# nucypher/TFHE.jl

Hardware: AMD Instinct MI355X
Metric: bootstrapped gates/sec (whole node), N=1024 (higher is better)
Workload: dtype int32 torus / f64 transform; 1 GPU; batch of 4096 independent gate_nand() bootstraps per GPU, tfhe_parameters_80 (n=500, N=1024, k=1, l=2, Bg=2^10, ks t=8, base 2^2); inputs=resident in HBM, launch=one process

## Files before the change

### tfhe.jl_amd/csrc/engine.hpp

```cpp
#pragma once
#include <hip/hip_runtime.h>

#include <algorithm>
#include <atomic>
#include <cstdarg>
#include <cstdio>
#include <cstring>
#include <new>
#include <string>
#include <thread>
#include <vector>

#include "../../include/tfhe_mi355x.h"
#include "experiment.hpp"
#include "br_core.hpp"

using namespace tfhe;

#include "kernels_blind_rotate.hpp"
#include "kernels_anyn.hpp"
#include "kernels_n512.hpp"
#include "kernels_keyswitch.hpp"

struct ErrBuf {
    char s[512] = {0};
    const char *c_str() const { return s; }
    void set(const char *msg) { snprintf(s, sizeof s, "%s", msg ? msg : ""); }
    ErrBuf &operator=(const char *msg) { set(msg); return *this; }
    void format(const char *fmt, ...) __attribute__((format(printf, 2, 3)))
    {
        va_list ap;
        va_start(ap, fmt);
        vsnprintf(s, sizeof s, fmt, ap);
        va_end(ap);
    }
};
extern thread_local ErrBuf g_create_error;

struct DevBuf {
    void *p = nullptr;
    size_t cap = 0;
    hipError_t reserve(size_t bytes)
    {
        if (bytes <= cap) return hipSuccess;
        if (p) (void)hipFree(p);
        p = nullptr; cap = 0;
        size_t want = bytes + bytes / 4 + 256;
        hipError_t e = hipMalloc(&p, want);
        if (e == hipSuccess) cap = want;
        return e;
    }
    void release() { if (p) (void)hipFree(p); p = nullptr; cap = 0; }
};

struct PairXfer {
    static constexpr int kSlots = 4;
    struct Slot {
        DevBuf out, idx_src;
        DevBuf in, idx_dst;
        int32_t *h_idx = nullptr; size_t h_idx_cap = 0;
        void *h_rows = nullptr; size_t h_rows_cap = 0;
        hipEvent_t ready = nullptr;
        hipEvent_t taken = nullptr;
        bool pending = false;
    } slot[kSlots];
    unsigned next = 0;
};

struct KsKey {
    int mode = 0;
    int parties = 1;
    int kN = 0;
    void *p = nullptr;
    size_t per_party = 0;
    int stride = 0;
    int wtiles = 0;
};
inline void release(KsKey &k)
{
    if (k.p) (void)hipFree(k.p);
    k = KsKey{};
}

struct tfhe_ctx {
    tfhe_params P{};
    int device = 0;
    ErrBuf err;
    std::vector<tfhe_ctx *> kids;
    std::vector<uint8_t> kid_ran;

    hipStream_t stream = nullptr;
    static constexpr int kTimingSlots = 33;
    hipEvent_t evring[kTimingSlots][4] = {};
    hipEvent_t *ev = evring[0];
    int64_t timed_calls = 0;
    hipEvent_t done_ev = nullptr;
    bool done_pending = false;
    bool timing_valid = false;
    bool own_pending = false;
    int64_t last_rotations = 0;
    std::string last_kernel;
    int ks_slices_large = 2;
    int ks_variant = 4;
    int64_t br_small = 1024;
    int br_prio_pct = 90;
    int br_general = 0;
    int br_split = 1;
    int timing_events = 1;
    int br_rt_l = 0;
    int64_t br_tiny = -2;

    cplx *d_tables = nullptr;
    Tables T{};
    Gadget g{};
    cplx *d_anyn_tab = nullptr;
    int br_anyn = 0;
    int anyn_spec = -1;
    bool anyn() const
    {
        if (br_anyn) return true;
        if (P.parties > 1) return P.N != kN || P.parties > 8 || P.bs_l > 8;
        if (n512()) return false;
        return (P.N != kN && P.N != 2048) || P.k > 4;
    }
    bool n512() const { return !br_anyn && P.parties == 1 && P.N == 512 && P.k == 1; }

    cplx *d_bk = nullptr;       size_t bk_polys = 0;
    KsKey ks;
    bool have_bk = false;
    bool have_ks() const { return ks.mode != 0 && ks.parties == 1; }
    cplx *d_mk_bk = nullptr;
    int mk_parties = 0;
    bool have_mk_bk = false;
    bool have_mk_ks() const { return ks.mode != 0 && ks.parties > 1; }

    int32_t *d_wires = nullptr; int64_t num_wires = 0;
    int wires_parties = 0;
    size_t wire_words() const { return wires_parties ? (size_t)wires_parties * P.n + 1 : (size_t)P.n + 1; }

    DevBuf bara, ext, map, io[4], diag, abar, mk_acc, spec;
    DevBuf tv, tv_index;
    DevBuf tv_bodies, tv_ext;
    cplx *d_tgsw = nullptr;        int64_t tgsw_count = 0;
    DevBuf lvl_ws[2], lvl_data, lvl_spec;
    cplx *d_mk_tgsw = nullptr;     int64_t mk_tgsw_count = 0;
    int32_t *d_mk_tgsw_party = nullptr;
    size_t diag_rows = 0;
    bool mk_force_general = false;
    int n2048_rw = 0;
    int mkg_rw = 0;
    int mkg_variant = 0;
    int mkg_acc = -1;
    int mk_rw = 0;
    bool measure_margin = false;
    int exact_domain = 2;
    double exact_bound_log2 = 0;
    double exact_margin = 0;
    tfhe_ctx *twin = nullptr;
    std::atomic<hipStream_t> twin_stream{nullptr};
    bool borrows_keys = false;
    bool slot_busy[2] = {false, false};
    std::atomic<std::thread::id> submit_thread{};
    uint32_t submits = 0;
    std::vector<std::vector<uint8_t>> wire_valid;
    std::vector<int32_t> wire_owner;
    std::vector<uint8_t> peer_ok;
    std::vector<struct PairXfer *> xfer;
    int level_exchange = 0;
    int64_t level_split_min = 4096;
    std::vector<int32_t> kid_tickets[2];
    int cu_count = 256;
    int w2_rw = 0;
    int n512_w2 = -1;
    int n512_rw = 0;
    int k2_w3 = -1;
    int k2_rw = 0;
    int v3_rw = 0;
    int64_t pipeline_min = 4096;
    bool last_call_two_streams = false;
    struct MapStage { void *h = nullptr; size_t cap = 0; hipEvent_t ev = nullptr; bool pending = false; };
    static constexpr int kMapStages = 4;
    MapStage map_stage[kMapStages];
    unsigned map_next = 0;
    MapStage *map_cur = &map_stage[0];
    void *h_map = nullptr;
// ... 71 lines not shown
constexpr size_t kTan2TableOffset = kN512TableOffset + kN512TableElems;

inline int ilog2i(int x) { int r = 0; while ((1 << r) < x) r++; return r; }
inline bool op_has_a(int op) { return !(op == TFHE_GATE_CONST0 || op == TFHE_GATE_CONST1); }
inline bool op_has_b(int op) { return op_has_a(op) && !(op == TFHE_GATE_NOT || op == TFHE_GATE_COPY); }
inline size_t bk_poly_count(const tfhe_params &p) { return (size_t)p.n * p.bs_l * (p.k + 1) * (p.k + 1); }

template <typename F>
struct ScopeExit {
    F f;
    ~ScopeExit() { f(); }
};
template <typename F>
ScopeExit<F> on_exit(F f) { return ScopeExit<F>{f}; }

template <typename F>
static int32_t fan_out(tfhe_ctx *c, const std::vector<int> &which, F &&fn)
{
    std::vector<int32_t> rcs(which.size(), TFHE_OK);
    std::vector<std::thread> th;
    std::vector<size_t> inline_ones;
    th.reserve(which.size());
    inline_ones.reserve(which.size());
    auto shard = [&](size_t i) noexcept {
        try { rcs[i] = fn(which[i]); } catch (...) { rcs[i] = abi_caught(c->kids[(size_t)which[i]], "fan-out shard"); }
    };
    for (size_t i = 1; i < which.size(); i++) {
        try {
            th.emplace_back([&shard, i] { shard(i); });
        } catch (...) {
            inline_ones.push_back(i);
        }
    }
    if (!which.empty()) shard(0);
    for (size_t i : inline_ones) shard(i);
    for (auto &t : th) t.join();
    std::fill(c->kid_ran.begin(), c->kid_ran.end(), 0);
    for (int k : which) c->kid_ran[(size_t)k] = 1;
    for (size_t i = 0; i < which.size(); i++)
        if (rcs[i]) return c->set_err(rcs[i], "device %d (kid %d): %s", c->kids[(size_t)which[i]]->device, which[i], c->kids[(size_t)which[i]]->err.c_str());
    return TFHE_OK;
}
inline std::vector<int> all_kids(const tfhe_ctx *c)
{
    std::vector<int> v(c->kids.size());
    for (size_t i = 0; i < v.size(); i++) v[i] = (int)i;
    return v;
}

template <typename F>
static int32_t multi_rows(tfhe_ctx *c, int64_t B, F &&call)
{
    const int nk = (int)c->kids.size();
    std::vector<int> which;
    std::vector<int64_t> lo((size_t)nk), hi((size_t)nk);
    for (int r = 0; r < nk; r++) {
        lo[(size_t)r] = B * r / nk; hi[(size_t)r] = B * (r + 1) / nk;
        if (hi[(size_t)r] > lo[(size_t)r]) which.push_back(r);
    }
    return fan_out(c, which, [&](int r) { return call(c->kids[(size_t)r], lo[(size_t)r], hi[(size_t)r] - lo[(size_t)r]); });
}

void shard_bounds_by_rotations(const uint8_t *opcodes, int64_t B, int shards, int64_t *bounds);
void quiesce(tfhe_ctx *c);
int32_t tgsw_prepare(tfhe_ctx *c, const int32_t *d_polys, cplx *d_out, size_t npolys, hipStream_t s);
void mk_tgsw_drop(tfhe_ctx *c);
struct DiagArgs;
int32_t prepare_diag(tfhe_ctx *c, size_t R, hipStream_t s, DiagArgs &d);
void name_kernel(tfhe_ctx *c, const char *fmt, ...) __attribute__((format(printf, 2, 3)));
struct TvPtrs { const int32_t *tv; const int32_t *index; int32_t *bodies = nullptr; int32_t n_out = 1; };
template <class A>
static WithTv<A> with_tv(const A &a, const TvPtrs &tv)
{
    WithTv<A> t;
    static_cast<A &>(t) = a;
    t.tv = tv.tv;
    t.tv_index = tv.index;
    t.bodies = tv.bodies;
    t.n_out = tv.n_out;
    return t;
}
int32_t launch_blind_rotate(tfhe_ctx *c, size_t R, int32_t mu, hipStream_t s, const TvPtrs *tv = nullptr);
int32_t launch_keyswitch(tfhe_ctx *c, size_t G, const int32_t *e0, const int32_t *e1, const int32_t *dst, const int32_t *ext, int32_t *out, hipStream_t s);
int32_t enter_stream(tfhe_ctx *c, hipStream_t s);
int32_t leave_stream(tfhe_ctx *c, hipStream_t s);
void next_timing_slot(tfhe_ctx *c);
void commit_timing_slot(tfhe_ctx *c);
int32_t ensure_host_map(tfhe_ctx *c, size_t bytes);
int32_t launch_prologue(tfhe_ctx *c, size_t R, const int32_t *d_in0, const int32_t *d_in1, const int32_t *d_in2, const int32_t *d_ra, const int32_t *d_rb,
                        const uint8_t *d_kind, int words, hipStream_t s);
int32_t run_gates(tfhe_ctx *c, const char *who, const uint8_t *opcodes, int64_t B, const int32_t *d_in0, const int32_t *d_in1, const int32_t *d_in2,
                  int32_t *d_out, const int32_t *ia, const int32_t *ib, const int32_t *ic, const int32_t *io, hipStream_t s);
int32_t launch_linear_prologue(tfhe_ctx *c, bool lut, size_t B, const int32_t *d_start, const int32_t *d_wire, const int32_t *d_coef,
                               const int32_t *d_cst, const int32_t *d_out, hipStream_t s);
struct IntLevel {
    const int32_t *tv; int32_t n_tv; const int32_t *tv_index; int32_t n_out;
    const int32_t *term_start, *term_wire, *term_coef, *cst, *out;
    int64_t B;
};
int32_t run_int_level(tfhe_ctx *c, const IntLevel &L);
int32_t launch_trivial(tfhe_ctx *c, size_t T, const int32_t *d_in0, const int32_t *d_ts, const int32_t *d_td, const uint8_t *d_top, int32_t *d_out,
                       int words, hipStream_t s);
int32_t launch_mk_blind_rotate(tfhe_ctx *c, size_t R, hipStream_t s, const TvPtrs *tv = nullptr);
int32_t mk_tv_launch_anyn(tfhe_ctx *c, const WithTv<anyn::Args> &a, unsigned nblk, unsigned nt, size_t lds, hipStream_t s);
int32_t mk_tv_launch_w2(tfhe_ctx *c, const WithTv<MkBrArgs> &a, int rw, unsigned nblk, size_t lds, hipStream_t s);
int32_t mk_tv_launch_general(tfhe_ctx *c, const WithTv<MkGenArgs> &a, int rw, bool accg, unsigned nblk, size_t lds, hipStream_t s);
int32_t run_mk_gates(tfhe_ctx *c, const char *who, const uint8_t *opcodes, int64_t B, const int32_t *d_in0, const int32_t *d_in1, const int32_t *d_in2,
                     int32_t *d_out, const int32_t *ia, const int32_t *ib, const int32_t *ic, const int32_t *io, hipStream_t s);
struct BrLaunch {
    int L;
    int rw;
    bool dg;
    dim3 grid, block;
    size_t lds;
};
int32_t br_launch_anyn(tfhe_ctx *c, const WithTv<anyn::Args> &a, const BrLaunch &g, hipStream_t s);
int32_t br_launch_n512w2(tfhe_ctx *c, const WithTv<N512Args> &a, const BrLaunch &g, hipStream_t s);
int32_t br_launch_n512(tfhe_ctx *c, const WithTv<N512Args> &a, const BrLaunch &g, hipStream_t s);
int32_t br_launch_general(tfhe_ctx *c, const WithTv<BrGenArgs> &a, bool n2048, const BrLaunch &g, hipStream_t s);
int32_t br_launch_n2048x(tfhe_ctx *c, const WithTv<Br2048Args> &a, const BrLaunch &g, hipStream_t s);
int32_t br_launch_k2w3(tfhe_ctx *c, const WithTv<BrArgs> &a, const BrLaunch &g, hipStream_t s);
int32_t br_launch_k2(tfhe_ctx *c, const WithTv<BrArgs> &a, const BrLaunch &g, hipStream_t s);
int32_t br_launch_h2(tfhe_ctx *c, const WithTv<BrArgs> &a, const H2Tables &ht, const BrLaunch &g, hipStream_t s);
int32_t br_launch_w2(tfhe_ctx *c, const WithTv<BrArgs> &a, const BrLaunch &g, hipStream_t s);
int32_t br_launch_v3(tfhe_ctx *c, const WithTv<BrArgs> &a, const BrLaunch &g, hipStream_t s);
struct LvlWant { DevBuf *buf; size_t bytes; };
int32_t leveled_reserve(tfhe_ctx *c, const char *who, const LvlWant *want, int count);
int32_t pull_wires(tfhe_ctx *c, int dst, const int32_t *wires, int64_t count);
```

### tfhe.jl_amd/csrc/engine_diag.hip

```cpp
#include "engine.hpp"

int32_t tfhe_last_timing_ms(tfhe_ctx *c, int32_t which, float *ms) try
{
    ENTER_CTX(c);
    if (!c || !ms) return TFHE_ERR_INVALID_ARG;
    if (c->multi()) {
        float worst = -1.f;
        for (size_t k = 0; k < c->kids.size(); k++) {
            if (!c->kid_ran[k]) continue;
            float v = 0.f;
            const int32_t rc = tfhe_last_timing_ms(c->kids[k], which, &v);
            if (rc) { c->err = c->kids[k]->err; return rc; }
            worst = v > worst ? v : worst;
        }
        if (worst < 0.f) return c->set_err(TFHE_ERR_STATE, "last_timing: no batch call recorded");
        *ms = worst;
        return TFHE_OK;
    }
    if (!c->timing_valid) return c->set_err(TFHE_ERR_STATE, "last_timing: no batch call recorded");
    HIP_TRY(c, hipSetDevice(c->device));
    HIP_TRY(c, hipEventSynchronize(c->ev[3]));
    int a, b;
    switch (which) {
    case 0: a = 1; b = 2; break;
// ... 121 lines not shown
    }
    return TFHE_OK;
}

int32_t tfhe_last_rounding_margin(tfhe_ctx *c, double *worst) try
{
    ENTER_CTX(c);
    if (!c || !worst) return TFHE_ERR_INVALID_ARG;
    if (c->multi()) {
        double m = -1;
        for (size_t k = 0; k < c->kids.size(); k++) {
            if (!c->kid_ran[k]) continue;
            double v = 0;
            const int32_t rc = read_diag(c->kids[k], &v, nullptr);
            if (rc) { c->err = c->kids[k]->err; return rc; }
            m = v > m ? v : m;
        }
        if (m < 0) return c->set_err(TFHE_ERR_STATE, "last_rounding_margin: no batch call recorded");
        *worst = m;
        return TFHE_OK;
    }
    return read_diag(c, worst, nullptr);
}
ABI_CATCH(c, "tfhe_last_rounding_margin")

int32_t tfhe_last_kernel_clock_mhz(tfhe_ctx *c, double *mhz) try
{
    ENTER_CTX(c);
    if (!c || !mhz) return TFHE_ERR_INVALID_ARG;
    if (c->multi()) {
        for (size_t k = 0; k < c->kids.size(); k++) {
            if (!c->kid_ran[k]) continue;
            const int32_t rc = read_diag(c->kids[k], nullptr, mhz);
            if (rc) c->err = c->kids[k]->err;
            return rc;
        }
        return c->set_err(TFHE_ERR_STATE, "last_kernel_clock: no batch call recorded");
    }
    return read_diag(c, nullptr, mhz);
}
ABI_CATCH(c, "tfhe_last_kernel_clock_mhz")

#ifdef TFHE_STAMP
extern "C" int32_t tfhe_debug_phases(tfhe_ctx *c, unsigned long long *out64)
{
    if (!c || !out64 || c->multi() || !c->diag_rows) return TFHE_ERR_STATE;
    HIP_TRY(c, hipSetDevice(c->device));
    HIP_TRY(c, hipDeviceSynchronize());
    HIP_TRY(c, hipMemcpyAsync(out64, (const char *)c->diag.p + c->diag_rows * 24, 64 * 8, hipMemcpyDeviceToHost, c->stream));
    HIP_TRY(c, hipStreamSynchronize(c->stream));
    return TFHE_OK;
}
#endif

int32_t tfhe_get_option(tfhe_ctx *c, const char *name, int64_t *value) try
{
    if (!c && name && value && !strcmp(name, "debug_fail_alloc_after")) { *value = g_fail_alloc_countdown.load(); return TFHE_OK; }
    ENTER_CTX(c);
    if (!name || !value) return c->set_err(TFHE_ERR_INVALID_ARG, "get_option: NULL argument");
    if (!strcmp(name, "exact_domain")) { *value = c->exact_domain; return TFHE_OK; }
    if (!strcmp(name, "exact_bound_log2_x1000")) { *value = (int64_t)std::llround(c->exact_bound_log2 * 1000.0); return TFHE_OK; }
    if (!strcmp(name, "exact_margin_x1e6")) { *value = (int64_t)std::llround(c->exact_margin * 1e6); return TFHE_OK; }
    if (!strcmp(name, "debug_fail_alloc_after")) { *value = g_fail_alloc_countdown.load(); return TFHE_OK; }
    if (c->multi() && !strcmp(name, "peer_pairs")) {
        int64_t n = 0;
        const size_t nk = c->kids.size();
        for (size_t a = 0; a < nk; a++)
            for (size_t b = 0; b < nk; b++) n += (a != b && c->peer_ok[a * nk + b]) ? 1 : 0;
        *value = n;
        return TFHE_OK;
    }
    if (c->multi() && strcmp(name, "level_split_min") && strcmp(name, "level_exchange")) {
        const int32_t rc = tfhe_get_option(c->kids[0], name, value);
        if (rc) c->err = c->kids[0]->err;
        return rc;
    }
    const struct { const char *n; int64_t v; } table[] = {
        {"br_small", c->br_small}, {"br_tiny", c->br_tiny}, {"br_rt_l", c->br_rt_l}, {"timing_events", c->timing_events},
        {"br_split", c->br_split}, {"br_general", c->br_general}, {"br_anyn", c->br_anyn}, {"anyn_spec", c->anyn_spec},
        {"level_split_min", c->level_split_min}, {"level_exchange", c->level_exchange}, {"br_prio_pct", c->br_prio_pct}, {"ks_slices", c->ks_slices_large},
        {"measure_margin", c->measure_margin ? 1 : 0}, {"pipeline_min", c->pipeline_min}, {"w2_rw", c->w2_rw}, {"k2_rw", c->k2_rw}, {"k2_w3", c->k2_w3}, {"n512_rw", c->n512_rw}, {"n512_w2", c->n512_w2},
        {"v3_rw", c->v3_rw}, {"mk_general", c->mk_force_general ? 1 : 0}, {"n2048_rw", c->n2048_rw}, {"mkg_acc", c->mkg_acc},
        {"mkg_variant", c->mkg_variant}, {"mkg_rw", c->mkg_rw}, {"mk_rw", c->mk_rw}, {"ks_variant", c->ks_variant},
    };
    for (const auto &e : table)
        if (!strcmp(name, e.n)) { *value = e.v; return TFHE_OK; }
    return c->set_err(TFHE_ERR_INVALID_ARG, "get_option: unknown option '%s'", name);
}
ABI_CATCH(c, "tfhe_get_option")

int32_t tfhe_set_option(tfhe_ctx *c, const char *name, int64_t value) try
{
    if (name && !strcmp(name, "debug_fail_alloc_after")) {
        if (value < 0) return TFHE_ERR_INVALID_ARG;
        g_fail_alloc_countdown.store(value);
        return TFHE_OK;
    }
    ENTER_CTX(c);
    if (!c) return TFHE_ERR_INVALID_ARG;
    if (!name || !*name) return TFHE_OK;
    if (c->multi()) {
        if (!strcmp(name, "level_split_min")) { c->level_split_min = value; return TFHE_OK; }
        if (!strcmp(name, "level_exchange")) {
            if (value < 0 || value > 2) return c->set_err(TFHE_ERR_INVALID_ARG, "set_option: level_exchange must be 0 (by peer access), 1 (device-to-device) or 2 (host staging)");
            c->level_exchange = (int)value;
            return TFHE_OK;
        }
        for (tfhe_ctx *k : c->kids) {
            const int32_t rc = tfhe_set_option(k, name, value);
            if (rc) { c->err = k->err; return rc; }
        }
        return TFHE_OK;
    }
    if (!strcmp(name, "br_small")) { c->br_small = value; return TFHE_OK; }
    if (!strcmp(name, "br_tiny")) { c->br_tiny = value; return TFHE_OK; }
    if (!strcmp(name, "br_rt_l")) { c->br_rt_l = value != 0; return TFHE_OK; }
    if (!strcmp(name, "timing_events")) { c->timing_events = value != 0; return TFHE_OK; }
    if (!strcmp(name, "br_split")) { c->br_split = value != 0; return TFHE_OK; }
    if (!strcmp(name, "br_general")) { c->br_general = value != 0; return TFHE_OK; }
    if (!strcmp(name, "br_anyn")) {
        if ((c->have_bk || c->have_mk_bk) && (value != 0) != (c->br_anyn != 0))
            return c->set_err(TFHE_ERR_STATE, "set_option: br_anyn must be chosen before the bootstrapping key is loaded (reload the key after changing it)");
        c->br_anyn = value != 0;
        return TFHE_OK;
    }
    if (!strcmp(name, "anyn_spec")) {
        if (value < -1 || value > 1) return c->set_err(TFHE_ERR_INVALID_ARG, "set_option: anyn_spec must be -1 (LDS when it fits), 0 (LDS) or 1 (global memory)");
        c->anyn_spec = (int)value;
        return TFHE_OK;
    }
    if (!strcmp(name, "level_split_min") || !strcmp(name, "level_exchange")) return TFHE_OK;
    if (!strcmp(name, "br_prio_pct")) {
        if (value < 0 || value > 100) return c->set_err(TFHE_ERR_INVALID_ARG, "set_option: br_prio_pct must be 0..100");
        c->br_prio_pct = (int)value;
        return TFHE_OK;
    }
    if (!strcmp(name, "ks_slices")) {
        if (value != 1 && value != 2 && value != 4) return c->set_err(TFHE_ERR_INVALID_ARG, "set_option: ks_slices must be 1, 2 or 4");
        c->ks_slices_large = (int)value;
        return TFHE_OK;
    }
    if (!strcmp(name, "measure_margin")) { c->measure_margin = value != 0; return TFHE_OK; }
    if (!strcmp(name, "pipeline_min")) { c->pipeline_min = value; return TFHE_OK; }
    if (!strcmp(name, "w2_rw")) {
        if (value < 0 || value > 2) return c->set_err(TFHE_ERR_INVALID_ARG, "set_option: w2_rw must be 0 (by batch size), 1 or 2");
        c->w2_rw = (int)value;
        return TFHE_OK;
    }
    if (!strcmp(name, "n512_w2")) {
        if (value < -1 || value > 1) return c->set_err(TFHE_ERR_INVALID_ARG, "set_option: n512_w2 must be -1 (by batch size), 0 (never) or 1 (always)");
        c->n512_w2 = (int)value;
        return TFHE_OK;
    }
    if (!strcmp(name, "n512_rw")) {
        if (value != 0 && value != 1 && value != 4) return c->set_err(TFHE_ERR_INVALID_ARG, "set_option: n512_rw must be 0 (by batch size), 1 or 4");
        c->n512_rw = (int)value;
        return TFHE_OK;
    }
    if (!strcmp(name, "k2_w3")) {
        if (value < -1 || value > 1) return c->set_err(TFHE_ERR_INVALID_ARG, "set_option: k2_w3 must be -1 (by batch size), 0 (never) or 1 (always)");
        c->k2_w3 = (int)value;
        return TFHE_OK;
    }
    if (!strcmp(name, "k2_rw")) {
        if (value != 0 && value != 1 && value != 7) return c->set_err(TFHE_ERR_INVALID_ARG, "set_option: k2_rw must be 0 (by batch size), 1 or 7");
        c->k2_rw = (int)value;
        return TFHE_OK;
    }
    if (!strcmp(name, "v3_rw")) {
        if (value != 0 && value != 1 && value != 4) return c->set_err(TFHE_ERR_INVALID_ARG, "set_option: v3_rw must be 0 (by batch size), 1 or 4");
        c->v3_rw = (int)value;
        return TFHE_OK;
    }
    if (!strcmp(name, "mk_general")) { c->mk_force_general = value != 0; return TFHE_OK; }
    if (!strcmp(name, "n2048_rw")) {
        if (value != 0 && value != 1 && value != 2) return c->set_err(TFHE_ERR_INVALID_ARG, "set_option: n2048_rw must be 0 (by batch size), 1 or 2");
        c->n2048_rw = (int)value;
        return TFHE_OK;
    }
    if (!strcmp(name, "mkg_acc")) {
        if (value < -1 || value > 1) return c->set_err(TFHE_ERR_INVALID_ARG, "set_option: mkg_acc must be -1 (by party count), 0 (LDS) or 1 (global memory)");
        c->mkg_acc = (int)value;
        return TFHE_OK;
    }
    if (!strcmp(name, "mkg_variant")) {
        if (value != 0 && value != 1) return c->set_err(TFHE_ERR_INVALID_ARG, "set_option: mkg_variant must be 0 (two-wave kernel for the shipped 4- / 8-party sets) or 1 (any-party kernel)");
        c->mkg_variant = (int)value;
        return TFHE_OK;
    }
    if (!strcmp(name, "mkg_rw")) {
        if (value != 0 && value != 1 && value != 2 && value != 4) return c->set_err(TFHE_ERR_INVALID_ARG, "set_option: mkg_rw must be 0 (by batch size), 1, 2 or 4 (4: the two-wave 4- / 8-party kernel only)");
        c->mkg_rw = (int)value;
        return TFHE_OK;
    }
    if (!strcmp(name, "mk_rw")) {
        if (value != 0 && value != 1 && value != 2) return c->set_err(TFHE_ERR_INVALID_ARG, "set_option: mk_rw must be 0 (by batch size), 1 or 2");
        c->mk_rw = (int)value;
        return TFHE_OK;
    }
    if (!strcmp(name, "ks_variant")) {
        if (value != 1 && value != 3 && value != 4) return c->set_err(TFHE_ERR_INVALID_ARG, "set_option: ks_variant must be 1, 3 or 4");
        if (c->ks.mode != 0 && (int)value != c->ks_variant)
            return c->set_err(TFHE_ERR_STATE, "set_option: ks_variant must be chosen before the keyswitch key is loaded (reload the key after changing it)");
        c->ks_variant = (int)value;
        return TFHE_OK;
    }
    return c->set_err(TFHE_ERR_INVALID_ARG, "set_option: unknown option '%s'", name);
}
ABI_CATCH(c, "tfhe_set_option")
```

### tfhe.jl_amd/csrc/engine_dispatch.hip

```cpp
#define TFHE_EMIT_KEYSWITCH_KERNELS
#include "engine.hpp"
#include "br_launch.hpp"

#include <map>
#include <mutex>
#include <functional>

int32_t ensure_dyn_lds(tfhe_ctx *c, const void *fn, size_t bytes, const char *what)
{
    static std::mutex mu;
    static std::map<std::pair<int, const void *>, size_t> have;
    std::lock_guard<std::mutex> lk(mu);
    size_t &cur = have[std::make_pair(c->device, fn)];
    if (cur >= bytes) return TFHE_OK;
    const hipError_t e = hipFuncSetAttribute(fn, hipFuncAttributeMaxDynamicSharedMemorySize, (int)bytes);
    if (e != hipSuccess) return c->set_err(TFHE_ERR_DEVICE, "hipFuncSetAttribute(%s, %zu bytes of LDS) failed: %s", what, bytes, hipGetErrorString(e));
    cur = bytes;
    return TFHE_OK;
}

int32_t prepare_diag(tfhe_ctx *c, size_t R, hipStream_t s, DiagArgs &d)
{
    d.margin_bits = nullptr; d.clk = nullptr; d.phase = nullptr;
    c->diag_rows = 0;
// ... 184 lines not shown
    if (q <= 7 && !allow_w3) return {{R, 0}};
    std::vector<double> best(q + 1, 1e300);
    std::vector<int> take(q + 1, 0);
    best[0] = 0.0;
    for (size_t i = 1; i <= q; i++)
        for (int n = 1; n <= 7 && (size_t)n <= i; n++)
            if (best[i - n] + kK2RoundCost[n] < best[i]) { best[i] = best[i - n] + kK2RoundCost[n]; take[i] = n; }
    int tail = 0;
    double total = best[q];
    for (int t = 1; allow_w3 && t <= 2 && (size_t)t <= q; t++)
        if (best[q - t] + kK2W3RoundCost[t] < total) { total = best[q - t] + kK2W3RoundCost[t]; tail = t; }
    std::vector<int> rounds;
    for (size_t i = q - (size_t)tail; i > 0; i -= (size_t)take[i]) rounds.push_back(take[i]);
    std::sort(rounds.begin(), rounds.end(), std::greater<int>());
    std::vector<K2Seg> seg;
    size_t done = 0;
    for (size_t i = 0; i < rounds.size() && done < R;) {
        size_t j = i;
        while (j < rounds.size() && rounds[j] == rounds[i]) j++;
        const size_t want = (size_t)rounds[i] * (j - i) * cus;
        if ((j == rounds.size() && !tail) || done + want >= R) { seg.push_back({R - done, 0}); done = R; break; }
        seg.push_back({want, 0});
        done += want;
        i = j;
    }
    if (done < R) seg.push_back({R - done, 1});
    return seg;
}

int32_t launch_blind_rotate(tfhe_ctx *c, size_t R, int32_t mu, hipStream_t s, const TvPtrs *tv)
{
    if (tv && c->measure_margin) return c->set_err(TFHE_ERR_STATE, "bootstrap_tv: no DIAG instantiation of the TV kernels (measure_margin is on)");
    DiagArgs diag;
    int32_t rc = prepare_diag(c, R, s, diag);
    if (rc) return rc;
    alloc_checkpoint();
    std::vector<K2Seg> seg;
    const bool tuned_l = c->P.bs_l == 2 || c->P.bs_l == 3;
    if (c->anyn()) {
    } else if (c->br_split && !c->br_general && !c->measure_margin && c->P.N == kN && c->P.k == 2 && tuned_l && (c->k2_rw == 0 || c->k2_rw == 7) && c->k2_w3 != 1) {
        seg = k2_partition(R, (size_t)c->cu_count, c->k2_w3 < 0);
    } else if (c->br_split && !c->br_general && c->P.N == kN && c->P.k == 1 && c->br_small > 0) {
        const size_t resident = 8 * (size_t)c->cu_count;
        if (R > resident && R % resident > 0 && R % resident <= (size_t)c->br_small) seg = {{R - R % resident, -1}, {R % resident, -1}};
    }
    auto part = [&](size_t first, size_t count, int kind) {
        const int32_t r = launch_blind_rotate_part(c, first, count, mu, s, diag, kind, tv);
        if (!r && tv) c->last_kernel += "+tv";
        return r;
    };
    if (seg.empty()) return part(0, R, -1);
    if (seg.size() == 1) return part(0, R, seg[0].kind);
    std::string names;
    size_t first = 0;
    for (const K2Seg &sg : seg) {
        rc = part(first, sg.count, sg.kind);
        if (rc) return rc;
        if (names.empty() || names.substr(names.rfind(" + ") == std::string::npos ? 0 : names.rfind(" + ") + 3) != c->last_kernel)
            names += (names.empty() ? "" : " + ") + c->last_kernel;
        first += sg.count;
    }
    c->last_kernel = names;
    return TFHE_OK;
}

template <class A>
static A ks_args(const tfhe_ctx *c, const int32_t *e0, const int32_t *e1, const int32_t *dst, const int32_t *ext, int32_t *out)
{
    const int P = c->ks.parties, kN = c->ks.kN, n = c->P.n;
    A a{};
    a.ext = ext; a.e0 = e0; a.e1 = e1; a.dst = dst; a.out = out;
    a.n = n; a.kN = kN;
    a.in_stride = P * kN + 1; a.in_off = 0; a.in_b = P * kN; a.out_stride = P * n + 1; a.out_off = 0; a.out_b = P * n;
    return a;
}

int32_t launch_keyswitch(tfhe_ctx *c, size_t G, const int32_t *e0, const int32_t *e1, const int32_t *dst, const int32_t *ext, int32_t *out, hipStream_t s)
{
    const KsKey &K = c->ks;
    const int P = K.parties, kN = K.kN, n = c->P.n;
    if (K.mode == 4) {
        Ks4Args a = ks_args<Ks4Args>(c, e0, e1, dst, ext, out);
        a.G = (int)G; a.wtiles = K.wtiles;
        a.kslices = (P > 1 || kN % 512 != 0) ? 1 : (G <= 512 ? 16 : c->ks_slices_large);
        if (a.kslices > 1) {
            const Ks3Args i3 = ks_args<Ks3Args>(c, e0, e1, dst, ext, out);
            hipLaunchKernelGGL(ks3_init_kernel, dim3((unsigned)G), dim3(256), 0, s, i3);
        }
        a.Gpad = (int)((G + 63) / 64 * 64);
        HIP_TRY(c, c->abar.reserve((size_t)(kN / 4) * a.Gpad * 16));
        a.abar_t = (const i32x4 *)c->abar.p;
        for (int p = 0; p < P; p++) {
            a.in_off = p * kN; a.out_off = p * n; a.add_b = (p == 0);
            a.bmat = (const i32x4 *)K.p + (size_t)p * K.per_party;
            hipLaunchKernelGGL(ks4_digits_kernel, dim3((unsigned)(a.Gpad / 32), (unsigned)(kN / 128)), dim3(128), 0, s, a, (i32x4 *)c->abar.p);
            hipLaunchKernelGGL(keyswitch_kernel_v4, dim3((unsigned)((G + 255) / 256), (unsigned)K.wtiles, (unsigned)a.kslices), dim3(256), 0, s, a);
        }
    } else if (K.mode == 3) {
        Ks3Args a = ks_args<Ks3Args>(c, e0, e1, dst, ext, out);
        a.t = c->P.ks_t; a.log2_base = 2; a.stride = K.stride; a.G = (int)G;
        a.ksp = (const int32_t *)K.p;
        hipLaunchKernelGGL(ks3_init_kernel, dim3((unsigned)G), dim3(256), 0, s, a);
        const unsigned tiles = (unsigned)((G + KS3_G - 1) / KS3_G);
        for (int p = 0; p < P; p++) {
            a.in_off = p * kN; a.out_off = p * n;
            a.ksp = (const int32_t *)K.p + (size_t)p * K.per_party;
            hipLaunchKernelGGL(keyswitch_kernel_v3, dim3(tiles * KS3_SLICES, (unsigned)((K.stride + 511) / 512)), dim3(128), 0, s, a);
        }
    } else {
        KsArgs a = ks_args<KsArgs>(c, e0, e1, dst, ext, out);
        a.t = c->P.ks_t; a.log2_base = c->P.ks_log2_base;
        for (int p = 0; p < P; p++) {
            a.in_off = p * kN; a.out_off = p * n; a.add_b = (p == 0);
            a.ks = (const int32_t *)K.p + (size_t)p * K.per_party;
            hipLaunchKernelGGL(keyswitch_kernel, dim3((unsigned)G, (unsigned)((n + 1 + 256 * KS1_WPT - 1) / (256 * KS1_WPT))), dim3(256), 0, s, a);
        }
    }
    HIP_TRY(c, hipGetLastError());
    return TFHE_OK;
}
```

### tfhe.jl_amd/csrc/engine_gates.hip

```cpp
#include "engine.hpp"
#include <chrono>
#include "kernels_gates.hpp"

int32_t enter_stream(tfhe_ctx *c, hipStream_t s)
{
    if (c->own_pending && s != c->stream) {
        HIP_TRY(c, hipEventRecord(c->done_ev, c->stream));
        c->own_pending = false;
        c->done_pending = true;
    }
    if (!c->done_pending) return TFHE_OK;
    const hipError_t q = hipEventQuery(c->done_ev);
    if (q == hipSuccess) { c->done_pending = false; return TFHE_OK; }
    if (q != hipErrorNotReady) return c->set_err(TFHE_ERR_DEVICE, "hipEventQuery failed: %s", hipGetErrorString(q));
    HIP_TRY(c, hipStreamWaitEvent(s, c->done_ev, 0));
    return TFHE_OK;
}
int32_t leave_stream(tfhe_ctx *c, hipStream_t s)
{
    if (s == c->stream) { c->own_pending = true; return TFHE_OK; }
    c->own_pending = false;
    HIP_TRY(c, hipEventRecord(c->done_ev, s));
    c->done_pending = true;
    return TFHE_OK;
// ... 128 lines not shown
    if (!no_ev) HIP_TRY(c, hipEventRecord(c->ev[3], s));
    if (Tn > 0) {
        hipLaunchKernelGGL(trivial_gates_kernel, dim3((unsigned)Tn), dim3(256), 0, s, d_in0, d_ts, d_td, d_top, d_out, n);
        HIP_TRY(c, hipGetLastError());
    }
    if (!no_ev) commit_timing_slot(c);
    c->last_rotations = (int64_t)R;
    MARK(7);
#ifdef TFHE_EXPERIMENT
    if (dbg_host) fprintf(stderr, "run_gates host us: classify+enter %.0f | stage %.0f | fill %.0f | map H2D %.0f | map event %.0f | prologue %.0f | blind rotate %.0f | keyswitch+trivial %.0f\n",
                          t_acc[0], t_acc[1], t_acc[2], t_acc[3], t_acc[4], t_acc[5], t_acc[6], t_acc[7]);
#endif
    return leave_stream(c, s);
}

int32_t launch_prologue(tfhe_ctx *c, size_t R, const int32_t *d_in0, const int32_t *d_in1, const int32_t *d_in2, const int32_t *d_ra, const int32_t *d_rb,
                        const uint8_t *d_kind, int words, hipStream_t s)
{
    hipLaunchKernelGGL(prologue_kernel, dim3((unsigned)R), dim3(256), 0, s, d_in0, d_in1, d_in2, d_ra, d_rb, d_kind, (int32_t *)c->bara.p, words, ilog2i(2 * c->P.N));
    HIP_TRY(c, hipGetLastError());
    return TFHE_OK;
}

int32_t launch_linear_prologue(tfhe_ctx *c, bool lut, size_t B, const int32_t *d_start, const int32_t *d_wire, const int32_t *d_coef,
                               const int32_t *d_cst, const int32_t *d_out, hipStream_t s)
{
    const int n = (int)c->wire_words() - 1, log2_2N = ilog2i(2 * c->P.N);
    if (lut)
        hipLaunchKernelGGL(linear_prologue_kernel<true>, dim3((unsigned)B), dim3(256), 0, s, (const int32_t *)c->d_wires, d_start, d_wire, d_coef,
                           d_cst, d_out, (int32_t *)c->bara.p, n, log2_2N);
    else
        hipLaunchKernelGGL(linear_prologue_kernel<false>, dim3((unsigned)B), dim3(256), 0, s, (const int32_t *)c->d_wires, d_start, d_wire, d_coef,
                           d_cst, d_out, c->d_wires, n, log2_2N);
    HIP_TRY(c, hipGetLastError());
    return TFHE_OK;
}

int32_t launch_trivial(tfhe_ctx *c, size_t T, const int32_t *d_in0, const int32_t *d_ts, const int32_t *d_td, const uint8_t *d_top, int32_t *d_out,
                       int words, hipStream_t s)
{
    hipLaunchKernelGGL(trivial_gates_kernel, dim3((unsigned)T), dim3(256), 0, s, d_in0, d_ts, d_td, d_top, d_out, words);
    HIP_TRY(c, hipGetLastError());
    return TFHE_OK;
}

int32_t tfhe_gates_batch_dev(tfhe_ctx *c, const uint8_t *opcodes, const int32_t *d_in0, const int32_t *d_in1,
                             const int32_t *d_in2, int32_t *d_out, int64_t B, void *stream) try
{
    ENTER_CTX(c);
    if (!c) return TFHE_ERR_INVALID_ARG;
    if (c->multi()) {
        if (c->kids.size() != 1) return c->set_err(TFHE_ERR_STATE, "gates_batch_dev: device pointers belong to one device; use tfhe_gates_batch on a multi-device context");
        const int32_t rc = tfhe_gates_batch_dev(c->kids[0], opcodes, d_in0, d_in1, d_in2, d_out, B, stream);
        if (rc) c->err = c->kids[0]->err;
        c->kid_ran[0] = 1;
        return rc;
    }
    if (B < 0 || (B > 0 && (!opcodes || !d_out))) return c->set_err(TFHE_ERR_INVALID_ARG, "gates_batch: NULL argument or negative B");
    if (B == 0) { c->timing_valid = false; c->last_rotations = 0; return TFHE_OK; }
    if (B > (int64_t)1 << 30) return c->set_err(TFHE_ERR_INVALID_ARG, "gates_batch: B too large");
    if (c->P.parties != 1) return c->set_err(TFHE_ERR_STATE, "gates_batch: context is multi-key");
    HIP_TRY(c, hipSetDevice(c->device));
    hipStream_t s = stream ? (hipStream_t)stream : c->stream;
    return run_gates(c, "gates_batch", opcodes, B, d_in0, d_in1, d_in2, d_out, nullptr, nullptr, nullptr, nullptr, s);
}
ABI_CATCH(c, "tfhe_gates_batch_dev")

static int32_t gates_batch_one_stream(tfhe_ctx *c, const uint8_t *opcodes, const int32_t *in0, const int32_t *in1, const int32_t *in2,
                                      int32_t *out, int64_t B, const bool (&need)[3]);

static int32_t ensure_twin(tfhe_ctx *c)
{
    if (!c->twin) {
        tfhe_ctx *t = nullptr;
        const int32_t rc = tfhe_ctx_create(&c->P, c->device, &t);
        if (rc) return c->set_err(rc, "gates_batch: second stream context: %s", g_create_error.c_str());
        t->borrows_keys = true;
        t->pipeline_min = -1;
        c->twin = t;
        c->twin_stream.store(t->stream, std::memory_order_release);
    }
    tfhe_ctx *t = c->twin;
    t->d_bk = c->d_bk; t->bk_polys = c->bk_polys; t->have_bk = c->have_bk; t->ks = c->ks;
    t->ks_slices_large = c->ks_slices_large; t->ks_variant = c->ks_variant; t->br_small = c->br_small; t->br_prio_pct = c->br_prio_pct;
    t->br_tiny = c->br_tiny; t->br_rt_l = c->br_rt_l; t->timing_events = c->timing_events; t->br_split = c->br_split; t->br_general = c->br_general; t->n2048_rw = c->n2048_rw; t->v3_rw = c->v3_rw; t->k2_rw = c->k2_rw; t->w2_rw = c->w2_rw;
    t->br_anyn = c->br_anyn; t->anyn_spec = c->anyn_spec; t->k2_w3 = c->k2_w3; t->n512_rw = c->n512_rw; t->n512_w2 = c->n512_w2;
    return TFHE_OK;
}

static int32_t multi_gates_batch(tfhe_ctx *c, const uint8_t *opcodes, const int32_t *in0, const int32_t *in1, const int32_t *in2,
                                 int32_t *out, int64_t B)
{
    const int nk = (int)c->kids.size();
    for (int64_t g = 0; g < B; g++)
        if (opcodes[g] >= TFHE_GATE__COUNT) return c->set_err(TFHE_ERR_INVALID_ARG, "gates_batch: bad opcode %d at gate %lld", opcodes[g], (long long)g);
    alloc_checkpoint();
    std::vector<int64_t> bounds((size_t)nk + 1);
    shard_bounds_by_rotations(opcodes, B, nk, bounds.data());
    std::vector<int> which;
    for (int r = 0; r < nk; r++)
        if (bounds[(size_t)r + 1] > bounds[(size_t)r]) which.push_back(r);
    const size_t n1 = (size_t)c->P.n + 1;
    return fan_out(c, which, [&](int r) {
        const int64_t s0 = bounds[(size_t)r], cnt = bounds[(size_t)r + 1] - s0;
        auto off = [&](const int32_t *p) { return p ? p + (size_t)s0 * n1 : nullptr; };
        return tfhe_gates_batch(c->kids[(size_t)r], opcodes + s0, off(in0), off(in1), off(in2), out + (size_t)s0 * n1, cnt);
    });
}

int32_t tfhe_gates_batch(tfhe_ctx *c, const uint8_t *opcodes, const int32_t *in0, const int32_t *in1,
                         const int32_t *in2, int32_t *out, int64_t B) try
{
    ENTER_CTX(c);
    if (!c) return TFHE_ERR_INVALID_ARG;
    if (B < 0 || (B > 0 && (!opcodes || !out))) return c->set_err(TFHE_ERR_INVALID_ARG, "gates_batch: NULL argument or negative B");
    if (B == 0) return TFHE_OK;
    if (c->multi()) return multi_gates_batch(c, opcodes, in0, in1, in2, out, B);
    HIP_TRY(c, hipSetDevice(c->device));
    bool need[3] = {false, false, false};
    for (int64_t g = 0; g < B; g++) {
        const int op = opcodes[g];
        if (op >= TFHE_GATE__COUNT) return c->set_err(TFHE_ERR_INVALID_ARG, "gates_batch: bad opcode %d at gate %lld", op, (long long)g);
        need[0] = need[0] || op_has_a(op); need[1] = need[1] || op_has_b(op); need[2] = need[2] || op == TFHE_GATE_MUX;
    }
    if ((need[0] && !in0) || (need[1] && !in1) || (need[2] && !in2))
        return c->set_err(TFHE_ERR_INVALID_ARG, "gates_batch: an operand array required by the opcodes is NULL");
    if (c->pipeline_min >= 0 && B >= c->pipeline_min && B >= 2 && !c->borrows_keys && !c->measure_margin && c->P.parties == 1 &&
        c->have_bk && c->have_ks()) {
        int64_t bounds[3];
        shard_bounds_by_rotations(opcodes, B, 2, bounds);
        if (c->P.N == kN && c->P.k == 1 && (c->P.bs_l == 2 || c->P.bs_l == 3) && !c->br_general && !c->anyn()) {
            const int64_t resident = 8 * (int64_t)c->cu_count;
            int64_t total = 0;
            for (int64_t g = 0; g < B; g++) total += opcodes[g] == TFHE_GATE_MUX ? 2 : op_has_b(opcodes[g]) ? 1 : 0;
            const int64_t target = (total / 2 + resident / 2) / resident * resident;
            if (target > 0 && target < total && total % resident != 0) {
                int64_t cum = 0, g = 0;
                while (g < B && cum < target) { cum += opcodes[g] == TFHE_GATE_MUX ? 2 : op_has_b(opcodes[g]) ? 1 : 0; g++; }
                if (cum == target || cum == target + 1) bounds[1] = g;
            }
        }
        if (bounds[1] > 0 && bounds[1] < B) {
            const int32_t rct = ensure_twin(c);
            if (rct) return rct;
            const size_t n1 = (size_t)c->P.n + 1;
            auto off = [&](const int32_t *p, int64_t g) { return p ? p + (size_t)g * n1 : nullptr; };
            const int64_t h = bounds[1];
            int32_t rc1 = TFHE_OK;
            std::thread second;
            try {
                second = std::thread([&] {
                    try { rc1 = gates_batch_one_stream(c->twin, opcodes + h, off(in0, h), off(in1, h), off(in2, h), out + (size_t)h * n1, B - h, need); }
                    catch (...) { rc1 = abi_caught(c->twin, "gates_batch (second half)"); }
                });
            } catch (const std::exception &) {
                return gates_batch_one_stream(c, opcodes, in0, in1, in2, out, B, need);
            }
            int32_t rc0;
            {
                auto joined = on_exit([&] { second.join(); });
                rc0 = gates_batch_one_stream(c, opcodes, in0, in1, in2, out, h, need);
            }
            if (rc1) return c->set_err(rc1, "gates_batch (second half): %s", c->twin->err.c_str());
            if (rc0) return rc0;
            c->last_rotations += c->twin->last_rotations;
            c->last_call_two_streams = true;
            return TFHE_OK;
// ... 414 lines not shown
```

### tfhe.jl_amd/csrc/kernels_keyswitch.hpp

```cpp
#pragma once
#include <hip/hip_runtime.h>

#include "../../include/tfhe_mi355x.h"
#include "br_core.hpp"

using namespace tfhe;

struct KsArgs {
    const int32_t *ext;
    const int32_t *ks;
    const int32_t *e0;
    const int32_t *e1;
    const int32_t *dst;
    int32_t *out;
    int32_t n, kN, t, log2_base;
    int32_t in_stride, in_off, in_b, out_stride, out_off, out_b;
    int32_t add_b;
};

constexpr int KS1_WPT = 4;

#ifdef TFHE_EMIT_KEYSWITCH_KERNELS
__global__ __launch_bounds__(256) void keyswitch_kernel(KsArgs P)
{
// ... 270 lines not shown
            for (int r = 0; r < 16; r++) acc[mt][pl][r] = 0;

    const size_t bstep = (size_t)P.wtiles * 4 * 64;
    const int i_begin = (int)blockIdx.z * (P.kN / P.kslices), i_end = i_begin + P.kN / P.kslices;
    const i32x4 *bp = P.bmat + (size_t)i_begin * bstep + ((size_t)wt * 4 + wave) * 64 + lane;
    const int stages = (i_end - i_begin) / 4;
    i32x4 pre[4];
#pragma unroll
    for (int ii = 0; ii < 4; ii++) bst[0][ii][wave][lane] = bp[(size_t)ii * bstep];

    i32x4 a_cur[MT], a_nxt[MT];
    auto load_a = [&](int i4, i32x4 (&a)[MT]) {
#pragma unroll
        for (int mt = 0; mt < MT; mt++) a[mt] = ap[mt][(size_t)(i4 >> 2) * P.Gpad];
    };
    load_a(i_begin, a_cur);

    for (int st = 0; st < stages; st++) {
        const bool more = st + 1 < stages;
        if (more) {
#pragma unroll
            for (int ii = 0; ii < 4; ii++) pre[ii] = bp[(size_t)(4 * (st + 1) + ii) * bstep];
            load_a(i_begin + 4 * (st + 1), a_nxt);
        }
        __syncthreads();
        if (wave_active) {
#pragma unroll
            for (int ii = 0; ii < 4; ii++) {
                i32x4 afrag[MT];
#pragma unroll
                for (int mt = 0; mt < MT; mt++)
#pragma unroll
                    for (int q = 0; q < 4; q++) {
                        const uint32_t d8 = ((uint32_t)a_cur[mt][ii] >> (27 - 2 * (4 * h + q))) & 24u;
                        afrag[mt][q] = (int32_t)(1u << d8);
                    }
#pragma unroll
                for (int pl = 0; pl < 4; pl++) {
                    const i32x4 bfrag = bst[st & 1][ii][pl][lane];
#pragma unroll
                    for (int mt = 0; mt < MT; mt++)
                        acc[mt][pl] = __builtin_amdgcn_mfma_i32_32x32x32_i8(afrag[mt], bfrag, acc[mt][pl], 0, 0, 0);
                }
            }
        }
        if (more) {
#pragma unroll
            for (int ii = 0; ii < 4; ii++) bst[(st + 1) & 1][ii][wave][lane] = pre[ii];
#pragma unroll
            for (int mt = 0; mt < MT; mt++) a_cur[mt] = a_nxt[mt];
        }
    }
    if (!wave_active) return;

    const int w = wt * 32 + c;
    if (w > P.n) return;
#pragma unroll
    for (int mt = 0; mt < MT; mt++)
#pragma unroll
        for (int r = 0; r < 16; r++) {
            const int gg = gbase + mt * 32 + (r & 3) + 8 * (r >> 2) + 4 * h;
            if (gg >= P.G) continue;
            uint32_t sum = (uint32_t)acc[mt][0][r] + ((uint32_t)acc[mt][1][r] << 8) + ((uint32_t)acc[mt][2][r] << 16) +
                           ((uint32_t)acc[mt][3][r] << 24);
            const size_t og = P.dst ? (size_t)P.dst[gg] : (size_t)gg;
            int32_t *o = P.out + og * P.out_stride;
            if (P.kslices > 1) {
                atomicAdd(reinterpret_cast<unsigned int *>(o + (w < P.n ? P.out_off + w : P.out_b)), 0u - sum);
            } else if (w < P.n) {
                o[P.out_off + w] = (int32_t)(0u - sum);
            } else {
                if (P.add_b) {
                    uint32_t b = (uint32_t)P.ext[(size_t)P.e0[gg] * P.in_stride + P.in_b];
                    const int e1 = P.e1 ? P.e1[gg] : -1;
                    if (e1 >= 0) b += (uint32_t)P.ext[(size_t)e1 * P.in_stride + P.in_b] + (1u << 29);
                    o[P.out_b] = (int32_t)(b - sum);
                } else {
                    o[P.out_b] = (int32_t)((uint32_t)o[P.out_b] - sum);
                }
            }
        }
}
#endif
```

Measured before the change: 355,700 gates/s.

## Add large-batch MFMA keyswitch kernel with LDS double-buffered key tiles

Adds a new keyswitch kernel for large batches (G >= 513 by default) that tiles several waves over gate groups and shares key-matrix fragments through double-buffered LDS. The global loads for the next stage are prefetched while the current stage's int8 MFMAs run. Block indices are remapped so neighbouring blocks share key tiles, which is meant to cut repeated key-matrix reads and raise MFMA utilisation compared with the v4 kernel. The change adds tuning knobs for the threshold and the tile shape, and brings more register pressure and a new code path.

Measured after the change: 355,200 gates/s. About the same (-0.1%).

```diff
diff --git a/tfhe.jl_amd/csrc/engine.hpp b/tfhe.jl_amd/csrc/engine.hpp
--- a/tfhe.jl_amd/csrc/engine.hpp
+++ b/tfhe.jl_amd/csrc/engine.hpp
@@ -101,6 +101,8 @@
     int64_t last_rotations = 0;
     std::string last_kernel;
     int ks_slices_large = 2;
+    int64_t ks_large_min = 513;
+    int ks_tile = 1;
     int ks_variant = 4;
     int64_t br_small = 1024;
     int br_prio_pct = 90;
@@ -338,6 +340,7 @@
 }
 int32_t launch_blind_rotate(tfhe_ctx *c, size_t R, int32_t mu, hipStream_t s, const TvPtrs *tv = nullptr);
 int32_t launch_keyswitch(tfhe_ctx *c, size_t G, const int32_t *e0, const int32_t *e1, const int32_t *dst, const int32_t *ext, int32_t *out, hipStream_t s);
+void launch_ks4_large(const Ks4Args &a, int tile, hipStream_t s);
 int32_t enter_stream(tfhe_ctx *c, hipStream_t s);
 int32_t leave_stream(tfhe_ctx *c, hipStream_t s);
 void next_timing_slot(tfhe_ctx *c);
diff --git a/tfhe.jl_amd/csrc/engine_diag.hip b/tfhe.jl_amd/csrc/engine_diag.hip
--- a/tfhe.jl_amd/csrc/engine_diag.hip
+++ b/tfhe.jl_amd/csrc/engine_diag.hip
@@ -227,6 +227,7 @@
         {"measure_margin", c->measure_margin ? 1 : 0}, {"pipeline_min", c->pipeline_min}, {"w2_rw", c->w2_rw}, {"k2_rw", c->k2_rw}, {"k2_w3", c->k2_w3}, {"n512_rw", c->n512_rw}, {"n512_w2", c->n512_w2},
         {"v3_rw", c->v3_rw}, {"mk_general", c->mk_force_general ? 1 : 0}, {"n2048_rw", c->n2048_rw}, {"mkg_acc", c->mkg_acc},
         {"mkg_variant", c->mkg_variant}, {"mkg_rw", c->mkg_rw}, {"mk_rw", c->mk_rw}, {"ks_variant", c->ks_variant},
+        {"ks_large_min", c->ks_large_min}, {"ks_tile", c->ks_tile},
     };
     for (const auto &e : table)
         if (!strcmp(name, e.n)) { *value = e.v; return TFHE_OK; }
@@ -285,6 +286,16 @@
         c->ks_slices_large = (int)value;
         return TFHE_OK;
     }
+    if (!strcmp(name, "ks_large_min")) {
+        if (value < 0) return c->set_err(TFHE_ERR_INVALID_ARG, "set_option: ks_large_min must be 0 (never) or a batch size");
+        c->ks_large_min = value;
+        return TFHE_OK;
+    }
+    if (!strcmp(name, "ks_tile")) {
+        if (value != 1 && value != 2) return c->set_err(TFHE_ERR_INVALID_ARG, "set_option: ks_tile must be 1 (<1, 8>) or 2 (<2, 4>)");
+        c->ks_tile = (int)value;
+        return TFHE_OK;
+    }
     if (!strcmp(name, "measure_margin")) { c->measure_margin = value != 0; return TFHE_OK; }
     if (!strcmp(name, "pipeline_min")) { c->pipeline_min = value; return TFHE_OK; }
     if (!strcmp(name, "w2_rw")) {
diff --git a/tfhe.jl_amd/csrc/engine_dispatch.hip b/tfhe.jl_amd/csrc/engine_dispatch.hip
--- a/tfhe.jl_amd/csrc/engine_dispatch.hip
+++ b/tfhe.jl_amd/csrc/engine_dispatch.hip
@@ -290,7 +290,9 @@
     if (K.mode == 4) {
         Ks4Args a = ks_args<Ks4Args>(c, e0, e1, dst, ext, out);
         a.G = (int)G; a.wtiles = K.wtiles;
-        a.kslices = (P > 1 || kN % 512 != 0) ? 1 : (G <= 512 ? 16 : c->ks_slices_large);
+        const bool sliceable = P == 1 && kN % 512 == 0;
+        const bool large = sliceable && c->ks_large_min > 0 && (int64_t)G >= c->ks_large_min;
+        a.kslices = !sliceable ? 1 : (large || G > 512) ? c->ks_slices_large : 16;
         if (a.kslices > 1) {
             const Ks3Args i3 = ks_args<Ks3Args>(c, e0, e1, dst, ext, out);
             hipLaunchKernelGGL(ks3_init_kernel, dim3((unsigned)G), dim3(256), 0, s, i3);
@@ -302,7 +304,8 @@
             a.in_off = p * kN; a.out_off = p * n; a.add_b = (p == 0);
             a.bmat = (const i32x4 *)K.p + (size_t)p * K.per_party;
             hipLaunchKernelGGL(ks4_digits_kernel, dim3((unsigned)(a.Gpad / 32), (unsigned)(kN / 128)), dim3(128), 0, s, a, (i32x4 *)c->abar.p);
-            hipLaunchKernelGGL(keyswitch_kernel_v4, dim3((unsigned)((G + 255) / 256), (unsigned)K.wtiles, (unsigned)a.kslices), dim3(256), 0, s, a);
+            if (large) launch_ks4_large(a, c->ks_tile, s);
+            else hipLaunchKernelGGL(keyswitch_kernel_v4, dim3((unsigned)((G + 255) / 256), (unsigned)K.wtiles, (unsigned)a.kslices), dim3(256), 0, s, a);
         }
     } else if (K.mode == 3) {
         Ks3Args a = ks_args<Ks3Args>(c, e0, e1, dst, ext, out);
diff --git a/tfhe.jl_amd/csrc/engine_gates.hip b/tfhe.jl_amd/csrc/engine_gates.hip
--- a/tfhe.jl_amd/csrc/engine_gates.hip
+++ b/tfhe.jl_amd/csrc/engine_gates.hip
@@ -234,7 +234,7 @@
     }
     tfhe_ctx *t = c->twin;
     t->d_bk = c->d_bk; t->bk_polys = c->bk_polys; t->have_bk = c->have_bk; t->ks = c->ks;
-    t->ks_slices_large = c->ks_slices_large; t->ks_variant = c->ks_variant; t->br_small = c->br_small; t->br_prio_pct = c->br_prio_pct;
+    t->ks_slices_large = c->ks_slices_large; t->ks_large_min = c->ks_large_min; t->ks_tile = c->ks_tile; t->ks_variant = c->ks_variant; t->br_small = c->br_small; t->br_prio_pct = c->br_prio_pct;
     t->br_tiny = c->br_tiny; t->br_rt_l = c->br_rt_l; t->timing_events = c->timing_events; t->br_split = c->br_split; t->br_general = c->br_general; t->n2048_rw = c->n2048_rw; t->v3_rw = c->v3_rw; t->k2_rw = c->k2_rw; t->w2_rw = c->w2_rw;
     t->br_anyn = c->br_anyn; t->anyn_spec = c->anyn_spec; t->k2_w3 = c->k2_w3; t->n512_rw = c->n512_rw; t->n512_w2 = c->n512_w2;
     return TFHE_OK;
diff --git a/tfhe.jl_amd/csrc/engine_ks_large.hip b/tfhe.jl_amd/csrc/engine_ks_large.hip
--- /dev/null
+++ b/tfhe.jl_amd/csrc/engine_ks_large.hip
@@ -0,0 +1,16 @@
+#define TFHE_EMIT_KS4_LARGE_KERNELS
+#include "engine.hpp"
+
+template <int MT, int WAVES>
+static void launch_tile(const Ks4Args &a, hipStream_t s)
+{
+    const int sgroups = (a.G + 32 * MT * WAVES - 1) / (32 * MT * WAVES);
+    const unsigned blocks = 8u * (unsigned)((sgroups + 1) / 2) * (unsigned)a.kslices * (unsigned)((a.wtiles + 3) / 4);
+    hipLaunchKernelGGL((ks4_large_kernel<MT, WAVES>), dim3(blocks), dim3(64 * WAVES), 0, s, a, sgroups);
+}
+
+void launch_ks4_large(const Ks4Args &a, int tile, hipStream_t s)
+{
+    if (tile == 2) launch_tile<2, 4>(a, s);
+    else launch_tile<1, 8>(a, s);
+}
diff --git a/tfhe.jl_amd/csrc/kernels_keyswitch.hpp b/tfhe.jl_amd/csrc/kernels_keyswitch.hpp
--- a/tfhe.jl_amd/csrc/kernels_keyswitch.hpp
+++ b/tfhe.jl_amd/csrc/kernels_keyswitch.hpp
@@ -376,3 +376,116 @@
         }
 }
 #endif
+
+#ifdef TFHE_EMIT_KS4_LARGE_KERNELS
+template <int MT, int WAVES>
+__global__ __launch_bounds__(64 * WAVES, WAVES == 4 ? 2 : 1) void ks4_large_kernel(Ks4Args P, int sgroups)
+{
+    constexpr int NF = 16 / WAVES;
+    __shared__ i32x4 bst[2][4][4][64];
+    const int lane = threadIdx.x & 63, wave = threadIdx.x >> 6;
+    const int c = lane & 31, h = lane >> 5;
+    const int lin = blockIdx.x;
+    const int cls = lin & 7, rest = lin >> 3;
+    const int sgh = (sgroups + 1) >> 1;
+    const int sg = 2 * (rest % sgh) + (cls & 1);
+    const int slice = (rest / sgh) % P.kslices;
+    const int wt = 4 * (rest / sgh / P.kslices) + (cls >> 1);
+    if (sg >= sgroups || wt >= P.wtiles) return;
+    const int gbase = (sg * WAVES + wave) * (32 * MT);
+    const bool wave_active = gbase < P.G;
+
+    const i32x4 *ap[MT];
+#pragma unroll
+    for (int mt = 0; mt < MT; mt++) ap[mt] = P.abar_t + min(gbase + mt * 32 + c, P.Gpad - 1);
+
+    i32x16 acc[MT][4];
+#pragma unroll
+    for (int mt = 0; mt < MT; mt++)
+#pragma unroll
+        for (int pl = 0; pl < 4; pl++)
+#pragma unroll
+            for (int r = 0; r < 16; r++) acc[mt][pl][r] = 0;
+
+    const size_t bstep = (size_t)P.wtiles * 4 * 64;
+    const int i_begin = slice * (P.kN / P.kslices), i_end = i_begin + P.kN / P.kslices;
+    const i32x4 *bp[NF];
+#pragma unroll
+    for (int f = 0; f < NF; f++) {
+        const int fi = wave + WAVES * f;
+        bp[f] = P.bmat + (size_t)(i_begin + (fi >> 2)) * bstep + ((size_t)wt * 4 + (fi & 3)) * 64 + lane;
+    }
+    const int stages = (i_end - i_begin) / 4;
+    i32x4 pre[NF];
+#pragma unroll
+    for (int f = 0; f < NF; f++) bst[0][(wave + WAVES * f) >> 2][(wave + WAVES * f) & 3][lane] = bp[f][0];
+
+    i32x4 a_cur[MT], a_nxt[MT];
+    auto load_a = [&](int i4, i32x4 (&a)[MT]) {
+#pragma unroll
+        for (int mt = 0; mt < MT; mt++) a[mt] = ap[mt][(size_t)(i4 >> 2) * P.Gpad];
+    };
+    load_a(i_begin, a_cur);
+
+    for (int st = 0; st < stages; st++) {
+        const bool more = st + 1 < stages;
+        if (more) {
+#pragma unroll
+            for (int f = 0; f < NF; f++) pre[f] = bp[f][(size_t)(4 * (st + 1)) * bstep];
+            load_a(i_begin + 4 * (st + 1), a_nxt);
+        }
+        __syncthreads();
+        if (wave_active) {
+#pragma unroll
+            for (int ii = 0; ii < 4; ii++) {
+                i32x4 afrag[MT];
+#pragma unroll
+                for (int mt = 0; mt < MT; mt++)
+#pragma unroll
+                    for (int q = 0; q < 4; q++) {
+                        const uint32_t d8 = ((uint32_t)a_cur[mt][ii] >> (27 - 2 * (4 * h + q))) & 24u;
+                        afrag[mt][q] = (int32_t)(1u << d8);
+                    }
+#pragma unroll
+                for (int pl = 0; pl < 4; pl++) {
+                    const i32x4 bfrag = bst[st & 1][ii][pl][lane];
+#pragma unroll
+                    for (int mt = 0; mt < MT; mt++)
+                        acc[mt][pl] = __builtin_amdgcn_mfma_i32_32x32x32_i8(afrag[mt], bfrag, acc[mt][pl], 0, 0, 0);
+                }
+            }
+        }
+        if (more) {
+#pragma unroll
+            for (int f = 0; f < NF; f++) bst[(st + 1) & 1][(wave + WAVES * f) >> 2][(wave + WAVES * f) & 3][lane] = pre[f];
+#pragma unroll
+            for (int mt = 0; mt < MT; mt++) a_cur[mt] = a_nxt[mt];
+        }
+    }
+    if (!wave_active) return;
+
+    const int w = wt * 32 + c;
+    if (w > P.n) return;
+#pragma unroll
+    for (int mt = 0; mt < MT; mt++)
+#pragma unroll
+        for (int r = 0; r < 16; r++) {
+            const int gg = gbase + mt * 32 + (r & 3) + 8 * (r >> 2) + 4 * h;
+            if (gg >= P.G) continue;
+            uint32_t sum = (uint32_t)acc[mt][0][r] + ((uint32_t)acc[mt][1][r] << 8) + ((uint32_t)acc[mt][2][r] << 16) +
+                           ((uint32_t)acc[mt][3][r] << 24);
+            const size_t og = P.dst ? (size_t)P.dst[gg] : (size_t)gg;
+            int32_t *o = P.out + og * P.out_stride;
+            if (P.kslices > 1) {
+                atomicAdd(reinterpret_cast<unsigned int *>(o + (w < P.n ? P.out_off + w : P.out_b)), 0u - sum);
+            } else if (w < P.n) {
+                o[P.out_off + w] = (int32_t)(0u - sum);
+            } else {
+                uint32_t b = (uint32_t)P.ext[(size_t)P.e0[gg] * P.in_stride + P.in_b];
+                const int e1 = P.e1 ? P.e1[gg] : -1;
+                if (e1 >= 0) b += (uint32_t)P.ext[(size_t)e1 * P.in_stride + P.in_b] + (1u << 29);
+                o[P.out_b] = (int32_t)(b - sum);
+            }
+        }
+}
+#endif
```
